# liruiluo/VLA-Adapter

Hardware: AMD Instinct MI355X
Metric: fine-tune samples/sec (224px img + 32-tok prompt), adapter-only, fwd+bwd+AdamW (higher is better)
Workload: dtype bf16

## Files before the change

include/vla_native.h:

```cpp
#ifndef VLA_NATIVE_H
#define VLA_NATIVE_H
#ifdef __cplusplus
extern "C" {
#endif

#define VLA_ERR_ARG (-1)
#define VLA_ERR_LAUNCH (-2)
#define VLA_ERR_UNSUPPORTED (-3)

#define VLA_ABI_VERSION 8
int vla_version(void);
int vla_desc_size(int which);
const char* vla_last_error(void);

enum { VLA_ACT_NONE = 0, VLA_ACT_GELU = 1, VLA_ACT_RELU = 2, VLA_ACT_GELU_TANH = 3, VLA_ACT_SWIGLU = 4, VLA_ACT_SWIGLU_BWD = 5 };

typedef struct vla_gemm_desc {
  const void* A;
  const void* B;
  void* C;
  const void* bias;
  const void* R;
  void* C2;
  int M, N, K, lda, ldb, ldc, ldr, ldc2;
  int res_mod;
  int act, batch;
  long long sA, sB, sC, sR, sC2, sBias;
  float alpha;
  int a_group, c_group;
  long long a_group_stride, c_group_stride;
  int rope_mode, rope_T, rope_dh, rope_cols;
  const float* rope_cos; const float* rope_sin;
  int r_group; long long r_group_stride;
  int c_live_mod, c_live_from;
  int split_k; float* ws;
  int bias_post_round;
  int fp8; const float* a_scale; const float* b_scale;
  const void* A2; const void* B2; int K2, lda2, ldb2;
} vla_gemm_desc;

enum {
  VLA_KERNEL_NT_SKINNY = 0,
  VLA_KERNEL_NT_64x128_S6 = 8,
  VLA_KERNEL_NT_128x128_S4 = 9,
  VLA_KERNEL_NT_128x128 = 10,
  VLA_KERNEL_NT_128x64 = 11,
  VLA_KERNEL_NT_256 = 12,
  VLA_KERNEL_TN_128 = 16,
  VLA_KERNEL_TN_256 = 17
};
int vla_gemm_nt_plan(const vla_gemm_desc* desc , int latency, int num_cus, int* split );
int vla_gemm_latency_hint(int on);
int vla_gemm256_extent_ok(const vla_gemm_desc* desc );
// ... 186 lines not shown
```

vla_adapter_amd/csrc/gemm.hip:

```cpp
#include <algorithm>
#include "gemm_epilogue.h"
#include "gemm_params.h"

namespace {

constexpr int BK = 64;
constexpr int EPI_PAD = 16;

__device__ __forceinline__ float apply_act(float v, int act) {
  switch (act) {
    case VLA_ACT_GELU: return rbf(gelu_erf(v));
    case VLA_ACT_RELU: return fmaxf(v, 0.f);
    case VLA_ACT_GELU_TANH: return rbf(gelu_tanh(v));
    default: return v;
  }
}

template <int BM, int BN, int STAGES, int WN = 2>
struct Cfg {
  static constexpr int NW = (BM / 64) * WN;
  static constexpr int NTHREADS = NW * 64;
  static constexpr int WTN = BN / WN;
  static constexpr int NT = WTN / 16;
  static constexpr int A_BYTES = BM * BK * 2, B_BYTES = BN * BK * 2;
  static constexpr int STAGE_BYTES = A_BYTES + B_BYTES;
  static constexpr int PIECES = STAGE_BYTES / 1024;
  static constexpr int PPW = PIECES / NW;
  static constexpr int EPI_STRIDE = WTN * 2 + EPI_PAD;
  static constexpr int LDS_BYTES = STAGES * STAGE_BYTES;
  static constexpr int NHALF = NW * 64 * EPI_STRIDE <= LDS_BYTES ? 1 : 2;
  static constexpr int EPI_ROWS = 64 / NHALF;
  static constexpr int EPI_BYTES = NW * EPI_ROWS * EPI_STRIDE;
  static_assert(EPI_BYTES <= LDS_BYTES, "epilogue staging must fit the operand ring");
  static_assert(PIECES % NW == 0, "pieces must divide evenly over the waves");
};

template <int BM, int BN, int STAGES, int ROPE, int WN = 2, bool F8 = false, bool EXT = false>
__global__ __launch_bounds__((BM / 64) * 64 * WN) __attribute__((amdgpu_waves_per_eu((F8 && EXT) ? 4 : 1)))
void gemm_nt_kernel(GemmP p) {
  using C = Cfg<BM, BN, STAGES, WN>;
  constexpr int EB = F8 ? 1 : 2;
  extern __shared__ __attribute__((aligned(16))) char smem[];
  const int tid = threadIdx.x, lane = tid & 63;
  const int wid = __builtin_amdgcn_readfirstlane(tid >> 6);
  const int wr = wid / WN, wc = wid - wr * WN;

  const int swz = xcd_order(blockIdx.x, p.ntiles);
  constexpr int GM = 6;
  const int tiles_m = p.ntiles / p.tiles_n, per_group = GM * p.tiles_n;
  const int grp = swz / per_group, rem = swz - grp * per_group;
  const int gm = min(GM, tiles_m - grp * GM);
  const int bm = grp * GM + rem % gm, bn = rem / gm;
  const int m0 = bm * BM, n0 = bn * BN;
  const int z = blockIdx.z;
  const char* Ab = reinterpret_cast<const char*>(p.A) + (long long)z * p.sA * EB;
  const char* Bb = reinterpret_cast<const char*>(p.B) + (long long)z * p.sB * EB;

  const int kc = ((lane & 7) ^ ((lane >> 3) & 7)) * 16;
  const char* pp[C::PPW];
#pragma unroll
  for (int i = 0; i < C::PPW; ++i) {
    const int pc = wid * C::PPW + i;
    if (pc < BM / 8) {
      const int ra = min(m0 + pc * 8 + (lane >> 3), p.M - 1);
      pp[i] = Ab + grouped_row(ra, p.gA, p.sgA, p.lda) * EB + kc;
    } else {
      const int rb = min(n0 + (pc - BM / 8) * 8 + (lane >> 3), p.N - 1);
      pp[i] = Bb + (long long)rb * p.ldb * EB + kc;
    }
  }
  const char* pp2[EXT ? C::PPW : 1];
  if constexpr (EXT) {
#pragma unroll
    for (int i = 0; i < C::PPW; ++i) {
      const int pc = wid * C::PPW + i;
      if (pc < BM / 8) pp2[i] = reinterpret_cast<const char*>(p.A2) + (long long)min(m0 + pc * 8 + (lane >> 3), p.M - 1) * p.lda2 * 2 + kc;
      else pp2[i] = reinterpret_cast<const char*>(p.B2) + (long long)min(n0 + (pc - BM / 8) * 8 + (lane >> 3), p.N - 1) * p.ldb2 * 2 + kc;
    }
  }
  const int nt1 = (p.Ktot > 0 ? min(p.K, p.Ktot - z * p.K) : p.K) / (F8 ? 2 * BK : BK);
  auto stage = [&](int buf, int t) {
    char* base = smem + buf * C::STAGE_BYTES + wid * C::PPW * 1024;
    if (EXT && t >= nt1) {
#pragma unroll
      for (int i = 0; i < C::PPW; ++i) glds16(pp2[i] + (t - nt1) * 128, base + i * 1024);
    } else {
#pragma unroll
      for (int i = 0; i < C::PPW; ++i) glds16(pp[i] + t * 128, base + i * 1024);
    }
  };

  f32x4 acc[C::NT][4];
#pragma unroll
  for (int a = 0; a < C::NT; ++a)
#pragma unroll
    for (int b = 0; b < 4; ++b) acc[a][b] = f32x4{0.f, 0.f, 0.f, 0.f};

  const int frow = lane & 15;
  int foff[2], foff2[2];
#pragma unroll
  for (int s = 0; s < 2; ++s) {
    foff[s] = frow * 128 + (((F8 ? 2 * (lane >> 4) + s : 4 * s + (lane >> 4)) ^ (lane & 7)) << 4);
    foff2[s] = frow * 128 + (((4 * s + (lane >> 4)) ^ (lane & 7)) << 4);
  }

  const int wm0 = m0 + wr * 64, wn0 = n0 + wc * C::WTN;
  const int lq = lane >> 4, lr = lane & 15;
  constexpr bool PERM = ROPE == 1 && C::NT == 2;
  const bool wide = PERM && p.rope_dh == 128;
  auto cbase = [&](int ni) { return PERM ? (wide ? ni * 64 + wc * 16 : (wc >> 1) * 64 + ni * 32 + (wc & 1) * 16) : wc * C::WTN + ni * 16; };
  const bf16_t* bias = p.bias ? p.bias + (long long)z * p.sBias : nullptr;
  float bv[C::NT][4];
  {
    const bool bvec = bias && (((size_t)bias & 7) == 0);
#pragma unroll
    for (int ni = 0; ni < C::NT; ++ni) {
      const int n = n0 + cbase(ni) + lq * 4;
      if (bvec && n + 3 < p.N) {
// ... 37 lines not shown
      _Pragma("unroll") for (int i = 0; i < C::NT; ++i) fn[s][i] = *reinterpret_cast<const bf16x8*>(sb + cbase(i) * 128 + FO[s]);    \
    }                                                                                                                                \
    if constexpr (F8T) {                                                                                                             \
      _Pragma("unroll") for (int ni = 0; ni < C::NT; ++ni)                                                                           \
        _Pragma("unroll") for (int mi = 0; mi < 4; ++mi)                                                                             \
          acc[ni][mi] = __builtin_amdgcn_mfma_scale_f32_16x16x128_f8f6f4(cat8(fn[0][ni], fn[1][ni]), cat8(fm[0][mi], fm[1][mi]),     \
                                                                         acc[ni][mi], 0, 0, 0, 0x7f7f7f7f, 0, 0x7f7f7f7f);            \
    } else {                                                                                                                         \
      _Pragma("unroll") for (int s = 0; s < 2; ++s)                                                                                  \
        _Pragma("unroll") for (int ni = 0; ni < C::NT; ++ni)                                                                         \
          _Pragma("unroll") for (int mi = 0; mi < 4; ++mi)                                                                           \
            acc[ni][mi] = __builtin_amdgcn_mfma_f32_16x16x32_bf16(fn[s][ni], fm[s][mi], acc[ni][mi], 0, 0, 0);                       \
    }                                                                                                                                \
    if (++buf == STAGES) buf = 0;                                                                                                    \
  } while (0)
  if constexpr (F8 && EXT) {
    for (int t = 0; t < nt1; ++t) VLA_KTILE(true, foff);
    {
      float fsa[4];
#pragma unroll
      for (int mi = 0; mi < 4; ++mi) fsa[mi] = p.scaleA[min(wm0 + mi * 16 + lr, p.M - 1)];
#pragma unroll
      for (int ni = 0; ni < C::NT; ++ni)
#pragma unroll
        for (int j = 0; j < 4; ++j) {
          const float sbv = p.scaleB[min(n0 + cbase(ni) + lq * 4 + j, p.N - 1)];
#pragma unroll
          for (int mi = 0; mi < 4; ++mi) acc[ni][mi][j] *= fsa[mi] * sbv;
        }
    }
    for (int t = nt1; t < nt; ++t) VLA_KTILE(false, foff2);
// ... 257 lines not shown
    for (int j = 0; j < 4; ++j) {
      float v = epi_linear(a[j], alpha, bias ? bb[j] : 0.f);
      if (act != VLA_ACT_NONE) v = apply_act(rbf(v), act);
      if (R) v = rbf(v) + rr[j];
      o[j] = v;
    }
    if (vec) {
      *reinterpret_cast<uint2*>(C + (long long)m * ldc + n) = pack4(o);
    } else {
#pragma unroll
      for (int j = 0; j < 4; ++j) C[(long long)m * ldc + n + j] = f2bf(o[j]);
    }
  }
}

template <int BM, int BN, int STAGES, int ROPE, int WN = 2, bool F8 = false, bool EXT = false>
int launch(const GemmP& p0, int nb, hipStream_t st) {
  using C = Cfg<BM, BN, STAGES, WN>;
  if (int rc = vla_lds_limit<gemm_nt_kernel<BM, BN, STAGES, ROPE, WN, F8, EXT>>(C::LDS_BYTES, "gemm_nt_kernel")) return rc;
  GemmP p = p0;
  p.tiles_n = (p.N + BN - 1) / BN;
  p.ntiles = ((p.M + BM - 1) / BM) * p.tiles_n;
  hipLaunchKernelGGL((gemm_nt_kernel<BM, BN, STAGES, ROPE, WN, F8, EXT>), dim3(p.ntiles, 1, nb), dim3(C::NTHREADS), C::LDS_BYTES, st, p);
  return VLA_OK;
}

template <int ROPE, bool F8 = false, bool EXT = false>
int launch_nt(int kernel, const GemmP& p, int nb, hipStream_t st) {
  if constexpr (!F8 && !EXT && ROPE != 3) {
    if (kernel == VLA_KERNEL_NT_64x128_S6) return launch<64, 128, 6, ROPE, 4>(p, nb, st);
    if (kernel == VLA_KERNEL_NT_128x128_S4) return launch<128, 128, 4, ROPE, 4>(p, nb, st);
    if constexpr (ROPE != 1)
      if (kernel == VLA_KERNEL_NT_128x64) return launch<128, 64, 2, ROPE>(p, nb, st);
  }
  return launch<128, 128, 2, ROPE, 4, F8, EXT>(p, nb, st);
}

struct NtOverrides {
// ... 48 lines not shown
      (d->rope_mode == 1 && d->rope_dh != 64) || !vla_gemm256_extent_ok(d))
    return false;
  const unsigned long long ra = (unsigned long long)((d->M + 255) / 256) * 256, rb = (unsigned long long)((d->N + 255) / 256) * 256;
  if ((ra * d->lda2 + d->K2) * 2 >= (1ull << 32) || (rb * d->ldb2 + d->K2) * 2 >= (1ull << 32)) return false;
  if (force != 0) return force == 6;
  const long long t256 = (long long)((d->M + 255) / 256) * ((d->N + 255) / 256);
  if (d->rope_mode == 1 && t256 < 192) return false;
  return use_256(d->M, d->N, d->K + d->K2, 1, d->act, ncu);
}

struct NtPlan { int kernel, split; };

NtPlan plan_nt(const vla_gemm_desc* d, bool latency, int ncu, const NtOverrides& ov) {
  const int force = ov.tile, kt = d->K / BK;
  const int asked = d->split_k > 1 ? d->split_k : 1, per = (kt + asked - 1) / asked, split = (kt + per - 1) / per;
  if (force == 0 && !ov.no_skinny && d->batch == 1 && split == 1 && d->a_group == 0 && d->c_group == 0 && d->r_group == 0 &&
      d->res_mod == 0 && d->c_live_mod == 0 && !d->fp8 && d->K2 == 0 && d->C) {
    const int t = skinny_tile(d, latency, ncu, ov.no_small_rows);
    if (t >= 0) return {VLA_KERNEL_NT_SKINNY + t, 1};
  }
  const bool fits256 = vla_gemm256_extent_ok(d) != 0;
  if (d->K2 > 0) return {!d->fp8 && ext_on_256(d, force, ncu) ? VLA_KERNEL_NT_256 : VLA_KERNEL_NT_128x128, 1};
  if (d->fp8) {
    const bool big = force == 6 || (force == 0 && d->M >= 4096 && d->N >= 4096 && d->K >= 4096);
    return {big && d->c_group == 0 && d->r_group == 0 && fits256 && !(d->rope_mode == 1 && d->rope_dh != 64) ? VLA_KERNEL_NT_256
                                                                                                              : VLA_KERNEL_NT_128x128, 1};
  }
  const int nb = asked > 1 ? asked : d->batch;
  bool square = false;
  if (asked == 1) {
// ... 104 lines not shown
  if (split_k) {
    VLA_REQUIRE(d->ws && d->batch == 1 && d->rope_mode == 0 && d->c_group == 0 && d->r_group == 0 &&
                    d->res_mod == 0 && d->c_live_mod == 0 && d->C &&
                    (d->act == VLA_ACT_NONE || d->act == VLA_ACT_GELU || d->act == VLA_ACT_RELU || d->act == VLA_ACT_GELU_TANH),
                "gemm: split_k needs an fp32 workspace [split_k, M, N], batch 1 and a plain epilogue");
    VLA_REQUIRE(d->N % 4 == 0 && ((uintptr_t)d->ws & 15) == 0, "gemm: split_k needs N % 4 == 0 and a 16-B aligned workspace");
  }
  VLA_REQUIRE(d->c_live_mod >= 0 && d->c_live_from >= 0 && (d->c_live_mod == 0 || d->c_live_from < d->c_live_mod),
              "gemm: c_live_from must lie inside c_live_mod");
  VLA_REQUIRE(d->r_group >= 0 && d->r_group_stride % 8 == 0 && (d->r_group == 0 || d->res_mod == 0),
              "gemm: r_group stride must keep 16-B alignment; r_group and res_mod are exclusive");
  if (d->K2 != 0)
    VLA_REQUIRE(d->K2 > 0 && d->K2 % BK == 0 && d->A2 && d->B2 && d->lda2 % 8 == 0 && d->ldb2 % 8 == 0 && (((uintptr_t)d->A2 | (uintptr_t)d->B2) & 15) == 0 &&
                    d->batch == 1 && !split_k && d->rope_mode != 2,
                "gemm: the K extension needs A2 / B2 (bf16, 16-B aligned rows, K2 % 64 == 0), batch 1, no split-K / interleaved RoPE");
  if (d->rope_mode != 0) {
    VLA_REQUIRE(d->rope_mode == 1 || d->rope_mode == 2, "gemm: rope_mode 0/1/2");
    VLA_REQUIRE(d->rope_cos && d->rope_sin && d->rope_T > 0 && d->rope_dh > 0 && d->rope_dh % 4 == 0 && d->rope_cols % 64 == 0 &&
                    (((uintptr_t)d->rope_cos | (uintptr_t)d->rope_sin) & 15) == 0 && d->act != VLA_ACT_SWIGLU,
                "gemm: bad rope arguments");
    if (d->rope_mode == 1) VLA_REQUIRE(d->rope_dh == 64 || (d->rope_dh == 128 && d->N % 128 == 0 && d->rope_cols % 128 == 0),
                                       "gemm: fused rotate_half RoPE needs head dim 64, or 128 with N and rope_cols multiples of 128");
  }

  const NtOverrides ov = nt_overrides();
  const int ncu = vla_num_cus();
  const NtPlan pl = plan_nt(d, g_latency_hint > 0, ncu, ov);

  GemmP p;
  p.A = (const bf16_t*)d->A; p.B = (const bf16_t*)d->B; p.C = (bf16_t*)d->C;
// ... 2 lines not shown
  p.ldc2 = d->ldc2; p.res_mod = d->res_mod; p.act = d->act;
  p.sA = d->sA; p.sB = d->sB; p.sC = d->sC; p.sR = d->sR; p.sC2 = d->sC2; p.sBias = d->sBias;
  p.tiles_n = p.ntiles = 0; p.batch = 1; p.stagger = 0;
  p.alpha = d->alpha == 0.f ? 1.f : d->alpha;
  p.gA = d->a_group; p.sgA = d->a_group_stride; p.gC = d->c_group; p.sgC = d->c_group_stride;
  p.gR = d->r_group; p.sgR = d->r_group_stride;
  p.c_live_mod = d->c_live_mod; p.c_live_from = d->c_live_from;
  p.bias_post = d->bias_post_round;
  p.ws = nullptr; p.Ktot = 0;
  if (split_k) {
    const int kt = d->K / BK;
    p.ws = d->ws;
    p.K = (kt + pl.split - 1) / pl.split * BK;
    p.Ktot = d->K;
    p.sA = p.sB = p.K;
    p.bias = nullptr; p.R = nullptr;
  }
  p.rope_mode = d->rope_mode; p.rope_T = d->rope_T; p.rope_dh = d->rope_dh; p.rope_cols = d->rope_cols;
  p.rope_cos = d->rope_cos; p.rope_sin = d->rope_sin;
  p.scaleA = d->fp8 ? d->a_scale : nullptr; p.scaleB = d->fp8 ? d->b_scale : nullptr;
  p.A2 = (const bf16_t*)d->A2; p.B2 = (const bf16_t*)d->B2; p.K2 = d->K2; p.lda2 = d->lda2; p.ldb2 = d->ldb2;

  hipStream_t st = (hipStream_t)stream;
  const int nb = pl.split > 1 ? pl.split : d->batch;
  const int rope = d->act == VLA_ACT_SWIGLU_BWD ? 3 : d->rope_mode;
  int rc;
  if (pl.kernel < VLA_KERNEL_NT_SKINNY + SKINNY_TILES) rc = vla_gemm_skinny_launch(p, pl.kernel - VLA_KERNEL_NT_SKINNY, st);
  else if (pl.kernel == VLA_KERNEL_NT_256)
    rc = vla_gemm256_launch(p, d->act == VLA_ACT_SWIGLU ? 1 : d->act == VLA_ACT_SWIGLU_BWD ? 2 : 0, d->batch, ov.grid_set ? ov.grid : ncu, st);
  else if (d->K2 > 0 && d->fp8)
    rc = rope == 3 ? launch_nt<3, true, true>(pl.kernel, p, nb, st) : rope == 1 ? launch_nt<1, true, true>(pl.kernel, p, nb, st)
                                                                                : launch_nt<0, true, true>(pl.kernel, p, nb, st);
  else if (d->K2 > 0)
    rc = rope == 3 ? launch_nt<3, false, true>(pl.kernel, p, nb, st) : rope == 1 ? launch_nt<1, false, true>(pl.kernel, p, nb, st)
                                                                                 : launch_nt<0, false, true>(pl.kernel, p, nb, st);
  else if (d->fp8) rc = rope == 1 ? launch_nt<1, true>(pl.kernel, p, nb, st) : launch_nt<0, true>(pl.kernel, p, nb, st);
  else if (rope == 3) rc = launch_nt<3>(pl.kernel, p, nb, st);
  else if (rope == 2) rc = launch_nt<2>(pl.kernel, p, nb, st);
  else if (rope == 1) rc = launch_nt<1>(pl.kernel, p, nb, st);
  else rc = launch_nt<0>(pl.kernel, p, nb, st);
  if (rc) return rc;
  VLA_CHECK_LAUNCH("gemm_bf16_nt");
  if (pl.split > 1) return splitk_finalize(d, pl.split, st);
  return VLA_OK;
}
```

vla_adapter_amd/engine.py:

```python
from __future__ import annotations

import contextlib
import math
import os
from dataclasses import dataclass, field
from typing import Dict, List, Optional, Tuple

import torch

from . import ops, schedule
from .ops import ACT_GELU, ACT_GELU_TANH, ACT_NONE, ACT_RELU, ACT_SWIGLU, BF16
from .schedule import Segment, capture_graph, chunks, turnaround_chunks

NUM_TOKENS = 64
IGNORE_INDEX = -100


def rup(n: int, m: int) -> int:
    return (n + m - 1) // m * m


def copy_flat(dst: torch.Tensor, src: torch.Tensor):
    n = src.numel()
    ops.copy2d(src, dst, 1, n, n, n)
# ... 557 lines not shown
        assert D % 64 == 0 and (D // self.H) % 8 == 0
        self.D, self.nb, self.Din = D, nb, Da * D
        assert self.Din % 64 == 0
        seg = [("w_adp", (nb, 2 * D, D)), ("b_adp", (nb, 2 * D)),
               ("w_task", (nb, 2 * D, D)), ("b_task", (nb, 2 * D))] if cfg.pro else []
        spec = [("w_x", (nb, 3 * D, D)), ("b_x", (nb, 3 * D))] + seg + [
                ("w_o", (nb, D, D)), ("b_o", (nb, D)), ("w_ffn", (nb, D, D)), ("b_ffn", (nb, D)),
                ("ln_w", (nb, D)), ("ln_b", (nb, D)), ("gate", (nb, 8)),
                ("ln1_w", (self.Din,)), ("ln1_b", (self.Din,)), ("fc1_w", (D, self.Din)), ("fc1_b", (D,)),
                ("ln2_w", (D,)), ("ln2_b", (D,)), ("fc2_w", (Da, D)), ("fc2_b", (Da,)),
                ("p_fc1_w", (D, Pd)), ("p_fc1_b", (D,)), ("p_fc2_w", (D, D)), ("p_fc2_b", (D,)),
                ("action_queries", (NUM_TOKENS, D))]
        self.P = FlatParams(spec, device)
        self.film = {}
        z = lambda *s: torch.zeros(*s, device=device, dtype=BF16)
        self.T = dict(w_x=z(nb, D, 3 * D), w_o=z(nb, D, D), w_ffn=z(nb, D, D), p_fc2_w=z(D, D))
        if cfg.pro:
            self.T.update(w_adp=z(nb, D, 2 * D), w_task=z(nb, D, 2 * D))
        self.fc2T = z(D, 64)
        self.pfc1_pad = z(D, 64)
        self.dirty = True
        self._key = None
        self._prep_key = None
        self.rope_tab = None
        self.ref_softmax = bool(int(os.environ.get("VLA_HEAD_REF_SOFTMAX", "0")))

    _BLK_PRO = [("q_proj", "w_x", "b_x", 0), ("k_self", "w_x", "b_x", 1), ("v_self", "w_x", "b_x", 2),
                ("k_adapter", "w_adp", "b_adp", 0), ("v_adapter", "w_adp", "b_adp", 1),
                ("k_task", "w_task", "b_task", 0), ("v_task", "w_task", "b_task", 1),
                ("o_proj", "w_o", "b_o", 0), ("ffn.1", "w_ffn", "b_ffn", 0)]
    _BLK_ORIG = [("q_proj", "w_x", "b_x", 0), ("k_proj", "w_x", "b_x", 1), ("v_proj", "w_x", "b_x", 2),
                 ("o_proj", "w_o", "b_o", 0), ("ffn.1", "w_ffn", "b_ffn", 0)]

    @property
    def _BLK(self):
        return self._BLK_PRO if self.pro else self._BLK_ORIG

    def _kv(self, which: str, i: int):
        D = self.D
        if self.pro:
            return self.P.view("w_" + which)[i], self.P.view("b_" + which)[i], self.T["w_" + which][i]
        return self.P.view("w_x")[i, D:], self.P.view("b_x")[i, D:], self.T["w_x"][i][:, D:]

    def named_views(self, buf=None) -> Dict[str, torch.Tensor]:
        P, D, out = self.P, self.D, {}
        v = lambda n: P.view(n, buf)
        for i in range(self.nb):
            pre = f"model.mlp_resnet_blocks.{i}."
            for name, w, b, k in self._BLK:
                out[pre + name + ".weight"] = v(w)[i, k * D:(k + 1) * D]
                out[pre + name + ".bias"] = v(b)[i, k * D:(k + 1) * D]
            out[pre + "ffn.0.weight"], out[pre + "ffn.0.bias"] = v("ln_w")[i], v("ln_b")[i]
            out[pre + "gating_factor"] = v("gate")[i, :1]
        for a, b in (("model.layer_norm1.weight", "ln1_w"), ("model.layer_norm1.bias", "ln1_b"), ("model.fc1.weight", "fc1_w"),
                     ("model.fc1.bias", "fc1_b"), ("model.layer_norm2.weight", "ln2_w"), ("model.layer_norm2.bias", "ln2_b"),
                     ("model.fc2.weight", "fc2_w"), ("model.fc2.bias", "fc2_b")):
            out[a] = v(b)
# ... 10 lines not shown
            t.copy_(head_sd[k].to(self.device, BF16).reshape(t.shape))
        for k, t in head_sd.items():
            if "film_gen" in k:
                self.film[k] = t.to(self.device, BF16)
        for k, t in self.proprio_views().items():
            t.copy_(proprio_sd[k].to(self.device, BF16))
        if action_queries is not None:
            self.P.view("action_queries").copy_(action_queries.to(self.device, BF16))
        self.dirty = True

    def head_state_dict(self):
        sd = {k: v.clone() for k, v in self.named_views().items()}
        sd.update(self.film)
        return sd

    @property
    def dirty(self) -> bool:
        return self._stale_fwd or self._stale_bwd

    @dirty.setter
    def dirty(self, v: bool):
        self._stale_fwd = self._stale_bwd = bool(v)

    def refresh_forward_operands(self):
        if self._stale_fwd:
            pd = self.cfg.proprio_dim
            ops.copy2d(self.P.view("p_fc1_w"), self.pfc1_pad, self.D, pd, pd, self.pfc1_pad.stride(0))
            self._stale_fwd = False

    def refresh_transposes(self):
        if not self._stale_bwd:
            return
        P = self.P
        for k in (("w_x", "w_adp", "w_task", "w_o", "w_ffn") if self.pro else ("w_x", "w_o", "w_ffn")):
            ops.transpose(P.view(k), out=self.T[k])
        ops.transpose(P.view("p_fc2_w"), out=self.T["p_fc2_w"])
        ops.transpose(P.view("fc2_w"), out=self.fc2T)
        self._stale_bwd = False

    def _alloc(self, B: int, Kt: int):
        if self._key == (B, Kt):
            return
        before = dict(self.__dict__)
        D, nb, T, dev = self.D, self.nb, self.cfg.chunk, self.device
        Ka = NUM_TOKENS + 1
        e = lambda *s, dt=BF16: torch.empty(*s, device=dev, dtype=dt)
        z = lambda *s, dt=BF16: torch.zeros(*s, device=dev, dtype=dt)
        R = B * T
        self.Ka, self.Kt, self.R = Ka, Kt, R
        self.h_adp = e(nb, B, Ka, D)
        self.KV_adp, self.KV_task = e(nb, B * Ka, 2 * D), e(nb, B * Kt, 2 * D)
        self.dKV_adp, self.dKV_task = e(nb, B * Ka, 2 * D), e(nb, B * Kt, 2 * D)
        self.X = e(nb + 1, R, D)
# ... 55 lines not shown
            assert tuple(noise.shape) == (T, self.Din) and noise.is_contiguous()
            ops.copy2d(noise, self.x_in, B * T, self.Din, self.Din, self.Din, src_mod=T)
        else:
            ops.zero_(self.x_in)
        self.x_ln, self.st1 = ops.layernorm_fwd(self.x_in, P.view("ln1_w"), P.view("ln1_b"), 1e-5, want_stats=True)
        ops.gemm_nt(self.x_ln, P.view("fc1_w"), bias=P.view("fc1_b"), act=ACT_RELU, out=self.X[0])

    def fwd_layer(self, i: int):
        cfg, P, D, H = self.cfg, self.P, self.D, self.H
        HS, B, S, Kt, Ka, T = self.HSref, self.B, self.S, self.Kt, self.Ka, cfg.chunk
        dh = D // H
        rc, rs_ = self.rope_tab
        hs2 = HS[i + 1].view(B * S, D)
        ops.gather_rows(hs2, self.row_idx_ka.view(-1), self.h_adp[i].view(B * Ka, D))
        fuse = self.pro and D % 64 == 0 and not os.environ.get("VLA_NO_KV_ROPE_FUSE")
        wa, ba, _ = self._kv("adp", i)
        ops.gemm_nt(self.h_adp[i].view(B * Ka, D), wa, bias=ba, out=self.KV_adp[i], rope=(2, rc, rs_, Ka, dh, D) if fuse else None)
        wt, bt, _ = self._kv("task", i)
        ops.gemm_nt(hs2[:B * Kt], wt, bias=bt, out=self.KV_task[i], a_group=(Kt, S * D), bias_post_round=B > 1,
                    rope=(2, rc, rs_, Kt, dh, D) if fuse else None)
        x = self.X[i]
        if self.pro:
            if not fuse:
                ops.rope_inter_(self.KV_adp[i][:, :D], rc, rs_, Ka, H, dh, 0)
                ops.rope_inter_(self.KV_task[i][:, :D], rc, rs_, Kt, H, dh, 0)
            ops.gemm_nt(x, P.view("w_x")[i], bias=P.view("b_x")[i], out=self.QKVx[i], rope=(2, rc, rs_, T, dh, 2 * D))
        else:
            ops.gemm_nt(x, P.view("w_x")[i], bias=P.view("b_x")[i], out=self.QKVx[i])
        self._attn(i, fwd=True)
        ops.gemm_nt(self.AOx[i], P.view("w_o")[i], bias=P.view("b_o")[i], residual=x, out=self.O2[i])
        ops.layernorm_fwd(self.O2[i], P.view("ln_w")[i], P.view("ln_b")[i], 1e-5, out=self.LNo[i], stats=self.stats[i])
        ops.gemm_nt(self.LNo[i], P.view("w_ffn")[i], bias=P.view("b_ffn")[i], act=ACT_RELU, out=self.X[i + 1])

# ... 28 lines not shown
            self.bwd_layer(i, dHS)
        self.bwd_end()

    def prep_backward(self, pos1: torch.Tensor, Np: int, B: int, S: int, row0: int, pos0=None, cnt0=None):
        self._alloc(B, Np)
        g = self.guard if pos0 is not None else None
        ops.head_index_prep(pos1, pos0 if pos0 is not None else pos1, cnt0 if cnt0 is not None else pos1, self._idx_scratch,
                            self.row_idx_live_ka, g, B, S, Np, row0)
        self._prep_key = (B, S, Np, row0)

    def bwd_begin(self, dpred: torch.Tensor, row0: int = 0):
        cfg, P, nb = self.cfg, self.P, self.nb
        R, Da = self.R, cfg.action_dim
        self.row0 = row0
        assert self._prep_key == (self.B, self.S, self.Np, row0), "prep_backward() first"
        self.refresh_transposes()
        ops.zero_(self.acc32)
        dp = dpred.reshape(R, Da)
        ops.zero_(self.dpad)
        ops.copy2d(dp, self.dpad, R, Da, Da, 64)
        ops.colsum_(dp, self.b_f32["fc2_b"])
        self._dw(self.dpad, self.xf_ln, out=self.dfc2)
        ops.copy2d(self.dfc2, P.g("fc2_w"), Da, self.D, self.D, self.D)
        d_ln2 = ops.gemm_nt(self.dpad, self.fc2T)
        self.dx = ops.layernorm_bwd(d_ln2, self.X[nb], P.view("ln2_w"), self.st2, self.ln2_dw, self.ln2_db)

    def bwd_layer(self, i: int, dHS: torch.Tensor):
        P, D = self.P, self.D
        B, S, Kt, Ka = self.B, self.S, self.Kt, self.Ka
        dff = self.dFF[i]
        ops.relu_bwd(self.dx, self.X[i + 1], out=dff)
        d_ln = ops.gemm_nt(dff, self.T["w_ffn"][i])
        do2 = self.dO2[i]
        ops.layernorm_bwd(d_ln, self.O2[i], P.view("ln_w")[i], self.stats[i], self.ln_dw[i], self.ln_db[i], out=do2)
        d_ao = ops.gemm_nt(do2, self.T["w_o"][i])
        self._attn(i, fwd=False, dout=d_ao)
        self.dx = ops.gemm_nt(self.dQKVx[i], self.T["w_x"][i], residual=do2)
        ops.gemm_nt(self.dKV_adp[i], self._kv("adp", i)[2], out=self.dh_adp[i])
        ops.scatter_add_rows(self.dh_adp[i], self.row_idx_live_ka.view(-1), dHS[i + 1].view(-1, D))
        if self.row0 == 0:
            ops.gemm_nt(self.dKV_task[i], self._kv("task", i)[2], out=dHS[i + 1].view(B * S, D)[:B * Kt], c_group=(Kt, S * D))

    def bwd_end(self):
        cfg, P, D, nb = self.cfg, self.P, self.D, self.nb
        B, Ka = self.B, self.Ka
        G = P.g
        dy1 = ops.relu_bwd(self.dx, self.X[0])
        ops.colsum_(dy1, self.b_f32["fc1_b"])
        self._dw(dy1, self.x_ln, out=G("fc1_w"))
        d_xln = ops.gemm_nt(dy1, self._t(P.view("fc1_w")))
        ops.layernorm_bwd(d_xln, self.x_in, P.view("ln1_w"), self.st1, self.ln1_dw, self.ln1_db, want_dx=False)
        ops.colsum_(self.dh_adp.view(nb, B, Ka, D)[:, :, NUM_TOKENS].transpose(0, 1), self.d_pf32)
        d_pf = ops.cast_f32_bf16(self.d_pf32)
        ops.colsum_(d_pf, self.b_f32["p_fc2_b"])
        self._dw(d_pf, self.pp_act, out=G("p_fc2_w"))
        d_act = ops.gemm_nt(d_pf, self.T["p_fc2_w"])
        d_pre = ops.gelu_bwd(d_act, self.pp_pre)
        ops.colsum_(d_pre, self.b_f32["p_fc1_b"])
        self._dw(d_pre, self.pr_in, out=self.dpfc1)
        ops.copy2d(self.dpfc1, G("p_fc1_w"), D, cfg.proprio_dim, 64, cfg.proprio_dim)
        Kt, S = self.Kt, self.S
        h_adp = self.h_adp.view(nb, B * Ka, D)
        if self.h_task_c is None:
            h_task, tg = self.HSref[1:nb + 1, 0, :Kt], (Kt, S * D)
        else:
            for i in range(nb):
                ops.copy_rows3d(self.HSref[i + 1], self.h_task_c[i], B, Kt, D, S * D, D, Kt * D, D)
            h_task, tg = self.h_task_c, None
        ops.gemm_tn(self.dQKVx, self.X[:nb], out=G("w_x"))
        ops.gemm_tn(self.dO2, self.AOx, out=G("w_o"))
        ops.gemm_tn(self.dFF, self.LNo, out=G("w_ffn"))
# ... 2 lines not shown
            ops.gemm_tn(self.dKV_adp, h_adp, out=G("w_adp"))
            ops.gemm_tn(self.dKV_task, h_task, out=G("w_task"), rows=B * Kt, b_group=tg)
            ops.colsum_(self.dKV_adp, self.b_f32["b_adp"]); ops.colsum_(self.dKV_task, self.b_f32["b_task"])
        else:
            gkv = G("w_x")[:, self.D:]
            ops.gemm_tn(self.dKV_adp, h_adp, out=gkv, accumulate=True)
            ops.gemm_tn(self.dKV_task, h_task, out=gkv, accumulate=True, rows=B * Kt, b_group=tg)
            bkv = self.b_f32["b_x"][:, self.D:]
            ops.colsum_(self.dKV_adp, bkv); ops.colsum_(self.dKV_task, bkv)
        for k, t in self.b_f32.items():
            ops.cast_f32_bf16(t, out=G(k))
        ops.cast_f32_bf16(self.ln_dw, out=G("ln_w")); ops.cast_f32_bf16(self.ln_db, out=G("ln_b"))
        ops.cast_f32_bf16(self.ln1_dw, out=G("ln1_w")); ops.cast_f32_bf16(self.ln1_db, out=G("ln1_b"))
        ops.cast_f32_bf16(self.ln2_dw, out=G("ln2_w")); ops.cast_f32_bf16(self.ln2_db, out=G("ln2_b"))
        ops.copy2d(self.dgate, G("gate"), nb, 1, 1, 8)

    def _t(self, w2d):
        return ops.transpose(w2d.contiguous())

    def _dw(self, dy, x, out=None):
        return ops.gemm_tn(dy, x, out=out, split=0)


class VLAEngine(schedule.StepControls):

    def __init__(self, cfg: VLACfg, weights: Dict, device="cuda"):
        self.cfg, self.device = cfg, device
        self.vits = [ViT(c, sd, device, j) for j, (c, sd) in enumerate(zip(cfg.vit, weights["vit"]))]
        self.llm = LLM(cfg.llm, weights["llm"], device)
        self.head = Head(cfg, device)
        self.head.load_state_dicts(weights["head"], weights["proprio"], weights.get("action_queries"))
        g = lambda k: weights["proj"][k].to(device=device, dtype=BF16).contiguous()
        self.proj = {k: g(k) for k in weights["proj"]}
# ... 518 lines not shown
            with torch.cuda.stream(hs):
                clip.sumsq(*r_head, gscale)
                head_summed.record(hs)
            clip.sumsq(*r_aq, gscale)
            cur.wait_event(head_summed)
            clip.finalise()
            finalised.record(cur)
            hs.wait_event(finalised)

        def adam(sl):
            args = (self.step_count, lr, beta1, beta2, eps, wd)
            if clip is None:
                ops.adamw_(P.data[sl], P.grad[sl], P.m[sl], P.v[sl], *args, gscale=gscale)
            else:
                ops.adamw_clipped_(P.data[sl], P.grad[sl], P.m[sl], P.v[sl], clip.coef, *args, gscale=gscale)
        with torch.cuda.stream(hs):
            adam(slice(None, aq_off))
            side_done = torch.cuda.Event()
            side_done.record()
        adam(slice(aq_off, None))
        if join:
            cur.wait_event(side_done)
        self.head.dirty = True

    def begin_validation(self):
        self.flush()
        if self._vis_ev is not None:
            torch.cuda.current_stream().wait_event(self._vis_ev)
        self.head.refresh_forward_operands()

    def end_validation(self):
        if self._g_vis is not None:
            self._launch_vision()

    def val_forward(self, batch: Dict[str, torch.Tensor], noise: Optional[torch.Tensor] = None) -> torch.Tensor:
# ... 19 lines not shown
```

vla_adapter_amd/native.py:

```python
from __future__ import annotations

import ctypes as C
import os
from typing import NamedTuple

_HERE = os.path.dirname(os.path.abspath(__file__))
LIB_PATH = (os.environ.get("VLA_NATIVE_LIB") or None) or os.path.join(_HERE, "libvla_native.so")

ACT_NONE, ACT_GELU, ACT_RELU, ACT_GELU_TANH, ACT_SWIGLU, ACT_SWIGLU_BWD = 0, 1, 2, 3, 4, 5
KERNEL_NT_SKINNY, KERNEL_NT_64x128_S6, KERNEL_NT_128x128_S4, KERNEL_NT_128x128, KERNEL_NT_128x64, KERNEL_NT_256 = 0, 8, 9, 10, 11, 12
KERNEL_TN_128, KERNEL_TN_256 = 16, 17
ABI_VERSION = 8


class NativeLibraryMissing(ImportError):
    pass


class GemmDesc(C.Structure):
    _fields_ = [("A", C.c_void_p), ("B", C.c_void_p), ("C", C.c_void_p), ("bias", C.c_void_p), ("R", C.c_void_p),
                ("C2", C.c_void_p),
                ("M", C.c_int), ("N", C.c_int), ("K", C.c_int), ("lda", C.c_int), ("ldb", C.c_int), ("ldc", C.c_int),
                ("ldr", C.c_int), ("ldc2", C.c_int), ("res_mod", C.c_int), ("act", C.c_int), ("batch", C.c_int),
                ("sA", C.c_longlong), ("sB", C.c_longlong), ("sC", C.c_longlong), ("sR", C.c_longlong),
                ("sC2", C.c_longlong), ("sBias", C.c_longlong), ("alpha", C.c_float),
                ("a_group", C.c_int), ("c_group", C.c_int), ("a_group_stride", C.c_longlong), ("c_group_stride", C.c_longlong),
                ("rope_mode", C.c_int), ("rope_T", C.c_int), ("rope_dh", C.c_int), ("rope_cols", C.c_int),
                ("rope_cos", C.c_void_p), ("rope_sin", C.c_void_p),
                ("r_group", C.c_int), ("r_group_stride", C.c_longlong), ("c_live_mod", C.c_int), ("c_live_from", C.c_int),
                ("split_k", C.c_int), ("ws", C.c_void_p), ("bias_post_round", C.c_int),
                ("fp8", C.c_int), ("a_scale", C.c_void_p), ("b_scale", C.c_void_p),
                ("A2", C.c_void_p), ("B2", C.c_void_p), ("K2", C.c_int), ("lda2", C.c_int), ("ldb2", C.c_int)]


class GemmTnDesc(C.Structure):
    _fields_ = [("A", C.c_void_p), ("B", C.c_void_p), ("C", C.c_void_p), ("R", C.c_void_p),
                ("M", C.c_int), ("N1", C.c_int), ("N2", C.c_int), ("lda", C.c_int), ("ldb", C.c_int), ("ldc", C.c_int),
                ("ldr", C.c_int), ("batch", C.c_int),
                ("sA", C.c_longlong), ("sB", C.c_longlong), ("sC", C.c_longlong), ("sR", C.c_longlong), ("alpha", C.c_float),
                ("a_group", C.c_int), ("b_group", C.c_int), ("a_group_stride", C.c_longlong), ("b_group_stride", C.c_longlong),
                ("a_col_group", C.c_int), ("a_col_group_stride", C.c_int), ("split", C.c_int), ("ws", C.c_void_p)]


class AttnDesc(C.Structure):
    _fields_ = [("q", C.c_void_p), ("k", C.c_void_p), ("v", C.c_void_p), ("o", C.c_void_p), ("lse", C.c_void_p),
                ("kmask", C.c_void_p),
                ("q_sb", C.c_longlong), ("k_sb", C.c_longlong), ("v_sb", C.c_longlong), ("o_sb", C.c_longlong),
# ... 211 lines not shown
```

vla_adapter_amd/ops.py:

```python
from __future__ import annotations

import ctypes as C
import math
from typing import Optional, Tuple

import torch

from . import native as N
from .native import ACT_GELU, ACT_GELU_TANH, ACT_NONE, ACT_RELU, ACT_SWIGLU, ACT_SWIGLU_BWD

BF16 = torch.bfloat16


def _lib():
    return N.load()


def _st():
    return C.c_void_p(torch.cuda.current_stream().cuda_stream)


def _p(t: Optional[torch.Tensor]):
    return None if t is None else C.c_void_p(t.data_ptr())


def _chk_bf16(*ts):
    for t in ts:
        if t is not None:
            assert t.is_cuda and t.dtype == BF16, f"expected CUDA bf16 tensor, got {t.device} {t.dtype}"


def gemm_nt(a: torch.Tensor, b: torch.Tensor, *, bias=None, residual=None, res_mod: int = 0, act: int = ACT_NONE,
            out: Optional[torch.Tensor] = None, out2: Optional[torch.Tensor] = None, alpha: float = 1.0,
            want_pre: bool = True, a_group=None, c_group=None, r_group=None, rope=None, c_live=None,
            split_k: Optional[int] = None, bias_post_round: bool = False, fp8=None, ext=None, query_256: bool = False,
            query_plan: bool = False):
    if fp8 is not None:
        assert a.dtype == torch.uint8 and b.dtype == torch.uint8 and a.dim() == 2 and split_k in (None, 0, 1)
        _chk_bf16(bias, residual, out, out2)
        split_k = 0
    else:
        _chk_bf16(a, b, bias, residual, out, out2)
    assert a.stride(-1) == 1 and b.stride(-1) == 1
    batched = a.dim() == 3
    if batched:
        nb, M, K = a.shape
        sA = a.stride(0)
        sB = b.stride(0) if b.dim() == 3 else 0
        Nn = b.shape[-2]
    else:
        nb, (M, K), sA, sB, Nn = 1, a.shape, 0, 0, b.shape[0]
    assert b.shape[-1] == K, f"K mismatch {a.shape} x {b.shape}"
    d = N.GemmDesc()
    d.A, d.B = a.data_ptr(), b.data_ptr()
    d.M, d.N, d.K, d.lda, d.ldb, d.batch = M, Nn, K, a.stride(-2), b.stride(-2), nb
    d.sA, d.sB, d.act, d.alpha, d.res_mod = sA, sB, act, alpha, res_mod
    shape = (nb, M, Nn) if batched else (M, Nn)
    if act == ACT_SWIGLU:
        if out is None and want_pre:
            out = torch.empty(shape, device=a.device, dtype=BF16)
        hshape = shape[:-1] + (Nn // 2,)
        if out2 is None:
            out2 = torch.empty(hshape, device=a.device, dtype=BF16)
        assert out2.shape == hshape and out2.stride(-1) == 1
        d.C2, d.ldc2, d.sC2 = out2.data_ptr(), out2.stride(-2), (out2.stride(0) if batched else 0)
    elif out is None:
        out = torch.empty(shape, device=a.device, dtype=BF16)
    if out is not None:
        assert tuple(out.shape) == tuple(shape) and out.stride(-1) == 1, f"out shape {out.shape} != {shape}"
        d.C, d.ldc, d.sC = out.data_ptr(), out.stride(-2), (out.stride(0) if batched else 0)
    if bias is not None:
# ... 1211 lines not shown
```

Baseline: 1367.

## Read [K,N] weights directly in backward GEMMs via transposing LDS loads

Adds a B_KN variant of the NT GEMM kernel that stages B tiles from a row-major [K, N] weight and uses ds_read_b64_tr_b16 transposing LDS reads to build MFMA operands. Backward data-gradient GEMMs now use the parameter views directly, so the per-step weight transposes and their transposed copies are removed. The b_kn path is pinned to a fixed 128x128 two-stage tile, which bypasses the planner's tile choice and may be slower for some shapes. Separately, the main-stream AdamW slice is now issued before the side-stream slice.

```diff
diff --git a/include/vla_native.h b/include/vla_native.h
--- a/include/vla_native.h
+++ b/include/vla_native.h
@@ -37,6 +37,7 @@
   int bias_post_round;
   int fp8; const float* a_scale; const float* b_scale;
   const void* A2; const void* B2; int K2, lda2, ldb2;
+  int b_kn;
 } vla_gemm_desc;
 
 enum {
diff --git a/vla_adapter_amd/csrc/gemm.hip b/vla_adapter_amd/csrc/gemm.hip
--- a/vla_adapter_amd/csrc/gemm.hip
+++ b/vla_adapter_amd/csrc/gemm.hip
@@ -14,6 +14,19 @@
     case VLA_ACT_GELU_TANH: return rbf(gelu_tanh(v));
     default: return v;
   }
+}
+
+template <int OFF>
+__device__ __forceinline__ bf16x8 lds_read16(unsigned addr) {
+  bf16x8 v;
+  asm volatile("ds_read_b128 %0, %1 offset:%2" : "=v"(v) : "v"(addr), "n"(OFF) : "memory");
+  return v;
+}
+template <int OFF>
+__device__ __forceinline__ bf16x4 lds_read_tr8(unsigned addr) {
+  bf16x4 v;
+  asm volatile("ds_read_b64_tr_b16 %0, %1 offset:%2" : "=v"(v) : "v"(addr), "n"(OFF) : "memory");
+  return v;
 }
 
 template <int BM, int BN, int STAGES, int WN = 2>
@@ -35,10 +48,11 @@
   static_assert(PIECES % NW == 0, "pieces must divide evenly over the waves");
 };
 
-template <int BM, int BN, int STAGES, int ROPE, int WN = 2, bool F8 = false, bool EXT = false>
+template <int BM, int BN, int STAGES, int ROPE, int WN = 2, bool F8 = false, bool EXT = false, bool B_KN = false>
 __global__ __launch_bounds__((BM / 64) * 64 * WN) __attribute__((amdgpu_waves_per_eu((F8 && EXT) ? 4 : 1)))
 void gemm_nt_kernel(GemmP p) {
   using C = Cfg<BM, BN, STAGES, WN>;
+  static_assert(!B_KN || (BN == 128 && ROPE == 0 && !F8 && !EXT), "B as [K, N]: plain bf16 products on 128-column tiles");
   constexpr int EB = F8 ? 1 : 2;
   extern __shared__ __attribute__((aligned(16))) char smem[];
   const int tid = threadIdx.x, lane = tid & 63;
@@ -64,6 +78,9 @@
     if (pc < BM / 8) {
       const int ra = min(m0 + pc * 8 + (lane >> 3), p.M - 1);
       pp[i] = Ab + grouped_row(ra, p.gA, p.sgA, p.lda) * EB + kc;
+    } else if constexpr (B_KN) {
+      const int r = (pc - BM / 8) * 4 + (lane >> 4), f = ((r & 3) << 2) | ((r >> 2) & 3);
+      pp[i] = Bb + ((long long)r * p.ldb + min(n0 + (((lane & 15) ^ f) << 3), p.N - 8)) * 2;
     } else {
       const int rb = min(n0 + (pc - BM / 8) * 8 + (lane >> 3), p.N - 1);
       pp[i] = Bb + (long long)rb * p.ldb * EB + kc;
@@ -84,6 +101,10 @@
     if (EXT && t >= nt1) {
 #pragma unroll
       for (int i = 0; i < C::PPW; ++i) glds16(pp2[i] + (t - nt1) * 128, base + i * 1024);
+    } else if constexpr (B_KN) {
+#pragma unroll
+      for (int i = 0; i < C::PPW; ++i)
+        glds16(pp[i] + (wid * C::PPW + i < BM / 8 ? (long long)t * 128 : (long long)t * BK * p.ldb * 2), base + i * 1024);
     } else {
 #pragma unroll
       for (int i = 0; i < C::PPW; ++i) glds16(pp[i] + t * 128, base + i * 1024);
@@ -102,6 +123,17 @@
   for (int s = 0; s < 2; ++s) {
     foff[s] = frow * 128 + (((F8 ? 2 * (lane >> 4) + s : 4 * s + (lane >> 4)) ^ (lane & 7)) << 4);
     foff2[s] = frow * 128 + (((4 * s + (lane >> 4)) ^ (lane & 7)) << 4);
+  }
+
+  int fbk[B_KN ? C::NT : 1][2];
+  if constexpr (B_KN) {
+    const int kq = lane >> 4, qq = (lane >> 2) & 3, pq = lane & 3;
+#pragma unroll
+    for (int e = 0; e < 2; ++e) {
+      const int row = 8 * kq + qq + 4 * e, f = (qq << 2) | ((2 * kq + e) & 3);
+#pragma unroll
+      for (int i = 0; i < C::NT; ++i) fbk[i][e] = 256 * row + ((((wc * C::WTN + i * 16) >> 3) + (pq >> 1)) ^ f) * 16 + 8 * (pq & 1);
+    }
   }
 
   const int wm0 = m0 + wr * 64, wn0 = n0 + wc * C::WTN;
@@ -169,7 +201,48 @@
     }                                                                                                                                \
     if (++buf == STAGES) buf = 0;                                                                                                    \
   } while (0)
-  if constexpr (F8 && EXT) {
+  if constexpr (B_KN) {
+    static_assert(!B_KN || STAGES == 2, "the [K, N] K loop is written for the two-stage ring");
+    const unsigned lds0 = (unsigned)(size_t)((__attribute__((address_space(3))) char*)smem);
+    for (int t = 0; t < nt; ++t) {
+      asm volatile("s_waitcnt vmcnt(0)" ::: "memory");
+      __builtin_amdgcn_s_barrier();
+      asm volatile("" ::: "memory");
+      if (t + 1 < nt) stage(buf ^ 1, t + 1);
+      const unsigned ua = lds0 + buf * C::STAGE_BYTES + wr * 64 * 128, ub = lds0 + buf * C::STAGE_BYTES + C::A_BYTES;
+      bf16x8 fm[2][4];
+      bf16x4 lo[2][C::NT], hi[2][C::NT];
+#pragma unroll
+      for (int s = 0; s < 2; ++s) {
+        const unsigned a0 = ua + foff[s];
+        fm[s][0] = lds_read16<0>(a0); fm[s][1] = lds_read16<2048>(a0); fm[s][2] = lds_read16<4096>(a0); fm[s][3] = lds_read16<6144>(a0);
+#pragma unroll
+        for (int i = 0; i < C::NT; ++i) {
+          if (s == 0) { lo[s][i] = lds_read_tr8<0>(ub + fbk[i][0]); hi[s][i] = lds_read_tr8<0>(ub + fbk[i][1]); }
+          else { lo[s][i] = lds_read_tr8<8192>(ub + fbk[i][0]); hi[s][i] = lds_read_tr8<8192>(ub + fbk[i][1]); }
+        }
+      }
+#pragma unroll
+      for (int s = 0; s < 2; ++s) {
+        static_assert(C::NT == 2, "the operand lists below name the two n tiles of a 64 x 32 wave tile");
+        if (s == 0)
+          asm volatile("s_waitcnt lgkmcnt(%8)" : "+v"(fm[0][0]), "+v"(fm[0][1]), "+v"(fm[0][2]), "+v"(fm[0][3]), "+v"(lo[0][0]), "+v"(hi[0][0]),
+                       "+v"(lo[0][1]), "+v"(hi[0][1]) : "n"(4 + 2 * C::NT) : "memory");
+        else
+          asm volatile("s_waitcnt lgkmcnt(0)" : "+v"(fm[1][0]), "+v"(fm[1][1]), "+v"(fm[1][2]), "+v"(fm[1][3]), "+v"(lo[1][0]), "+v"(hi[1][0]),
+                       "+v"(lo[1][1]), "+v"(hi[1][1]) : "v"(acc[0][0]), "v"(acc[0][1]), "v"(acc[0][2]), "v"(acc[0][3]), "v"(acc[1][0]),
+                       "v"(acc[1][1]), "v"(acc[1][2]), "v"(acc[1][3]) : "memory");
+        __builtin_amdgcn_sched_barrier(0);
+#pragma unroll
+        for (int ni = 0; ni < C::NT; ++ni) {
+          const bf16x8 fn = {lo[s][ni][0], lo[s][ni][1], lo[s][ni][2], lo[s][ni][3], hi[s][ni][0], hi[s][ni][1], hi[s][ni][2], hi[s][ni][3]};
+#pragma unroll
+          for (int mi = 0; mi < 4; ++mi) acc[ni][mi] = __builtin_amdgcn_mfma_f32_16x16x32_bf16(fn, fm[s][mi], acc[ni][mi], 0, 0, 0);
+        }
+      }
+      buf ^= 1;
+    }
+  } else if constexpr (F8 && EXT) {
     for (int t = 0; t < nt1; ++t) VLA_KTILE(true, foff);
     {
       float fsa[4];
@@ -457,14 +530,14 @@
   }
 }
 
-template <int BM, int BN, int STAGES, int ROPE, int WN = 2, bool F8 = false, bool EXT = false>
+template <int BM, int BN, int STAGES, int ROPE, int WN = 2, bool F8 = false, bool EXT = false, bool B_KN = false>
 int launch(const GemmP& p0, int nb, hipStream_t st) {
   using C = Cfg<BM, BN, STAGES, WN>;
-  if (int rc = vla_lds_limit<gemm_nt_kernel<BM, BN, STAGES, ROPE, WN, F8, EXT>>(C::LDS_BYTES, "gemm_nt_kernel")) return rc;
+  if (int rc = vla_lds_limit<gemm_nt_kernel<BM, BN, STAGES, ROPE, WN, F8, EXT, B_KN>>(C::LDS_BYTES, "gemm_nt_kernel")) return rc;
   GemmP p = p0;
   p.tiles_n = (p.N + BN - 1) / BN;
   p.ntiles = ((p.M + BM - 1) / BM) * p.tiles_n;
-  hipLaunchKernelGGL((gemm_nt_kernel<BM, BN, STAGES, ROPE, WN, F8, EXT>), dim3(p.ntiles, 1, nb), dim3(C::NTHREADS), C::LDS_BYTES, st, p);
+  hipLaunchKernelGGL((gemm_nt_kernel<BM, BN, STAGES, ROPE, WN, F8, EXT, B_KN>), dim3(p.ntiles, 1, nb), dim3(C::NTHREADS), C::LDS_BYTES, st, p);
   return VLA_OK;
 }
 
@@ -543,6 +616,7 @@
 NtPlan plan_nt(const vla_gemm_desc* d, bool latency, int ncu, const NtOverrides& ov) {
   const int force = ov.tile, kt = d->K / BK;
   const int asked = d->split_k > 1 ? d->split_k : 1, per = (kt + asked - 1) / asked, split = (kt + per - 1) / per;
+  if (d->b_kn) return {VLA_KERNEL_NT_128x128, split};
   if (force == 0 && !ov.no_skinny && d->batch == 1 && split == 1 && d->a_group == 0 && d->c_group == 0 && d->r_group == 0 &&
       d->res_mod == 0 && d->c_live_mod == 0 && !d->fp8 && d->K2 == 0 && d->C) {
     const int t = skinny_tile(d, latency, ncu, ov.no_small_rows);
@@ -677,6 +751,8 @@
     VLA_REQUIRE(d->K2 > 0 && d->K2 % BK == 0 && d->A2 && d->B2 && d->lda2 % 8 == 0 && d->ldb2 % 8 == 0 && (((uintptr_t)d->A2 | (uintptr_t)d->B2) & 15) == 0 &&
                     d->batch == 1 && !split_k && d->rope_mode != 2,
                 "gemm: the K extension needs A2 / B2 (bf16, 16-B aligned rows, K2 % 64 == 0), batch 1, no split-K / interleaved RoPE");
+  VLA_REQUIRE(d->b_kn == 0 || (d->b_kn == 1 && !d->fp8 && d->K2 == 0 && d->rope_mode == 0 && d->act != VLA_ACT_SWIGLU_BWD && d->N % 8 == 0),
+              "gemm: b_kn (B as [K, N]) needs N % 8 == 0, bf16 operands and no K extension / RoPE / SwiGLU backward");
   if (d->rope_mode != 0) {
     VLA_REQUIRE(d->rope_mode == 1 || d->rope_mode == 2, "gemm: rope_mode 0/1/2");
     VLA_REQUIRE(d->rope_cos && d->rope_sin && d->rope_T > 0 && d->rope_dh > 0 && d->rope_dh % 4 == 0 && d->rope_cols % 64 == 0 &&
@@ -709,6 +785,7 @@
     p.K = (kt + pl.split - 1) / pl.split * BK;
     p.Ktot = d->K;
     p.sA = p.sB = p.K;
+    if (d->b_kn) p.sB = (long long)p.K * d->ldb;
     p.bias = nullptr; p.R = nullptr;
   }
   p.rope_mode = d->rope_mode; p.rope_T = d->rope_T; p.rope_dh = d->rope_dh; p.rope_cols = d->rope_cols;
@@ -730,6 +807,7 @@
     rc = rope == 3 ? launch_nt<3, false, true>(pl.kernel, p, nb, st) : rope == 1 ? launch_nt<1, false, true>(pl.kernel, p, nb, st)
                                                                                  : launch_nt<0, false, true>(pl.kernel, p, nb, st);
   else if (d->fp8) rc = rope == 1 ? launch_nt<1, true>(pl.kernel, p, nb, st) : launch_nt<0, true>(pl.kernel, p, nb, st);
+  else if (d->b_kn) rc = launch<128, 128, 2, 0, 4, false, false, true>(p, nb, st);
   else if (rope == 3) rc = launch_nt<3>(pl.kernel, p, nb, st);
   else if (rope == 2) rc = launch_nt<2>(pl.kernel, p, nb, st);
   else if (rope == 1) rc = launch_nt<1>(pl.kernel, p, nb, st);
diff --git a/vla_adapter_amd/engine.py b/vla_adapter_amd/engine.py
--- a/vla_adapter_amd/engine.py
+++ b/vla_adapter_amd/engine.py
@@ -595,10 +595,7 @@
         self.P = FlatParams(spec, device)
         self.film = {}
         z = lambda *s: torch.zeros(*s, device=device, dtype=BF16)
-        self.T = dict(w_x=z(nb, D, 3 * D), w_o=z(nb, D, D), w_ffn=z(nb, D, D), p_fc2_w=z(D, D))
-        if cfg.pro:
-            self.T.update(w_adp=z(nb, D, 2 * D), w_task=z(nb, D, 2 * D))
-        self.fc2T = z(D, 64)
+        self.fc2_pad = z(64, D)
         self.pfc1_pad = z(D, 64)
         self.dirty = True
         self._key = None
@@ -620,8 +617,8 @@
     def _kv(self, which: str, i: int):
         D = self.D
         if self.pro:
-            return self.P.view("w_" + which)[i], self.P.view("b_" + which)[i], self.T["w_" + which][i]
-        return self.P.view("w_x")[i, D:], self.P.view("b_x")[i, D:], self.T["w_x"][i][:, D:]
+            return self.P.view("w_" + which)[i], self.P.view("b_" + which)[i]
+        return self.P.view("w_x")[i, D:], self.P.view("b_x")[i, D:]
 
     def named_views(self, buf=None) -> Dict[str, torch.Tensor]:
         P, D, out = self.P, self.D, {}
@@ -662,29 +659,15 @@
         sd.update(self.film)
         return sd
 
-    @property
-    def dirty(self) -> bool:
-        return self._stale_fwd or self._stale_bwd
-
-    @dirty.setter
-    def dirty(self, v: bool):
-        self._stale_fwd = self._stale_bwd = bool(v)
-
     def refresh_forward_operands(self):
-        if self._stale_fwd:
-            pd = self.cfg.proprio_dim
+        if self.dirty:
+            pd, Da = self.cfg.proprio_dim, self.cfg.action_dim
             ops.copy2d(self.P.view("p_fc1_w"), self.pfc1_pad, self.D, pd, pd, self.pfc1_pad.stride(0))
-            self._stale_fwd = False
+            ops.copy2d(self.P.view("fc2_w"), self.fc2_pad, Da, self.D, self.D, self.D)
+            self.dirty = False
 
     def refresh_transposes(self):
-        if not self._stale_bwd:
-            return
-        P = self.P
-        for k in (("w_x", "w_adp", "w_task", "w_o", "w_ffn") if self.pro else ("w_x", "w_o", "w_ffn")):
-            ops.transpose(P.view(k), out=self.T[k])
-        ops.transpose(P.view("p_fc2_w"), out=self.T["p_fc2_w"])
-        ops.transpose(P.view("fc2_w"), out=self.fc2T)
-        self._stale_bwd = False
+        self.refresh_forward_operands()
 
     def _alloc(self, B: int, Kt: int):
         if self._key == (B, Kt):
@@ -770,9 +753,9 @@
         hs2 = HS[i + 1].view(B * S, D)
         ops.gather_rows(hs2, self.row_idx_ka.view(-1), self.h_adp[i].view(B * Ka, D))
         fuse = self.pro and D % 64 == 0 and not os.environ.get("VLA_NO_KV_ROPE_FUSE")
-        wa, ba, _ = self._kv("adp", i)
+        wa, ba = self._kv("adp", i)
         ops.gemm_nt(self.h_adp[i].view(B * Ka, D), wa, bias=ba, out=self.KV_adp[i], rope=(2, rc, rs_, Ka, dh, D) if fuse else None)
-        wt, bt, _ = self._kv("task", i)
+        wt, bt = self._kv("task", i)
         ops.gemm_nt(hs2[:B * Kt], wt, bias=bt, out=self.KV_task[i], a_group=(Kt, S * D), bias_post_round=B > 1,
                     rope=(2, rc, rs_, Kt, dh, D) if fuse else None)
         x = self.X[i]
@@ -831,7 +814,6 @@
         R, Da = self.R, cfg.action_dim
         self.row0 = row0
         assert self._prep_key == (self.B, self.S, self.Np, row0), "prep_backward() first"
-        self.refresh_transposes()
         ops.zero_(self.acc32)
         dp = dpred.reshape(R, Da)
         ops.zero_(self.dpad)
@@ -839,7 +821,7 @@
         ops.colsum_(dp, self.b_f32["fc2_b"])
         self._dw(self.dpad, self.xf_ln, out=self.dfc2)
         ops.copy2d(self.dfc2, P.g("fc2_w"), Da, self.D, self.D, self.D)
-        d_ln2 = ops.gemm_nt(self.dpad, self.fc2T)
+        d_ln2 = ops.gemm_nt(self.dpad, self.fc2_pad, b_kn=True)
         self.dx = ops.layernorm_bwd(d_ln2, self.X[nb], P.view("ln2_w"), self.st2, self.ln2_dw, self.ln2_db)
 
     def bwd_layer(self, i: int, dHS: torch.Tensor):
@@ -847,16 +829,16 @@
         B, S, Kt, Ka = self.B, self.S, self.Kt, self.Ka
         dff = self.dFF[i]
         ops.relu_bwd(self.dx, self.X[i + 1], out=dff)
-        d_ln = ops.gemm_nt(dff, self.T["w_ffn"][i])
+        d_ln = ops.gemm_nt(dff, P.view("w_ffn")[i], b_kn=True)
         do2 = self.dO2[i]
         ops.layernorm_bwd(d_ln, self.O2[i], P.view("ln_w")[i], self.stats[i], self.ln_dw[i], self.ln_db[i], out=do2)
-        d_ao = ops.gemm_nt(do2, self.T["w_o"][i])
+        d_ao = ops.gemm_nt(do2, P.view("w_o")[i], b_kn=True)
         self._attn(i, fwd=False, dout=d_ao)
-        self.dx = ops.gemm_nt(self.dQKVx[i], self.T["w_x"][i], residual=do2)
-        ops.gemm_nt(self.dKV_adp[i], self._kv("adp", i)[2], out=self.dh_adp[i])
+        self.dx = ops.gemm_nt(self.dQKVx[i], P.view("w_x")[i], residual=do2, b_kn=True)
+        ops.gemm_nt(self.dKV_adp[i], self._kv("adp", i)[0], out=self.dh_adp[i], b_kn=True)
         ops.scatter_add_rows(self.dh_adp[i], self.row_idx_live_ka.view(-1), dHS[i + 1].view(-1, D))
         if self.row0 == 0:
-            ops.gemm_nt(self.dKV_task[i], self._kv("task", i)[2], out=dHS[i + 1].view(B * S, D)[:B * Kt], c_group=(Kt, S * D))
+            ops.gemm_nt(self.dKV_task[i], self._kv("task", i)[0], out=dHS[i + 1].view(B * S, D)[:B * Kt], c_group=(Kt, S * D), b_kn=True)
 
     def bwd_end(self):
         cfg, P, D, nb = self.cfg, self.P, self.D, self.nb
@@ -865,13 +847,13 @@
         dy1 = ops.relu_bwd(self.dx, self.X[0])
         ops.colsum_(dy1, self.b_f32["fc1_b"])
         self._dw(dy1, self.x_ln, out=G("fc1_w"))
-        d_xln = ops.gemm_nt(dy1, self._t(P.view("fc1_w")))
+        d_xln = ops.gemm_nt(dy1, P.view("fc1_w"), b_kn=True)
         ops.layernorm_bwd(d_xln, self.x_in, P.view("ln1_w"), self.st1, self.ln1_dw, self.ln1_db, want_dx=False)
         ops.colsum_(self.dh_adp.view(nb, B, Ka, D)[:, :, NUM_TOKENS].transpose(0, 1), self.d_pf32)
         d_pf = ops.cast_f32_bf16(self.d_pf32)
         ops.colsum_(d_pf, self.b_f32["p_fc2_b"])
         self._dw(d_pf, self.pp_act, out=G("p_fc2_w"))
-        d_act = ops.gemm_nt(d_pf, self.T["p_fc2_w"])
+        d_act = ops.gemm_nt(d_pf, P.view("p_fc2_w"), b_kn=True)
         d_pre = ops.gelu_bwd(d_act, self.pp_pre)
         ops.colsum_(d_pre, self.b_f32["p_fc1_b"])
         self._dw(d_pre, self.pr_in, out=self.dpfc1)
@@ -904,9 +886,6 @@
         ops.cast_f32_bf16(self.ln1_dw, out=G("ln1_w")); ops.cast_f32_bf16(self.ln1_db, out=G("ln1_b"))
         ops.cast_f32_bf16(self.ln2_dw, out=G("ln2_w")); ops.cast_f32_bf16(self.ln2_db, out=G("ln2_b"))
         ops.copy2d(self.dgate, G("gate"), nb, 1, 1, 8)
-
-    def _t(self, w2d):
-        return ops.transpose(w2d.contiguous())
 
     def _dw(self, dy, x, out=None):
         return ops.gemm_tn(dy, x, out=out, split=0)
@@ -1455,11 +1434,11 @@
                 ops.adamw_(P.data[sl], P.grad[sl], P.m[sl], P.v[sl], *args, gscale=gscale)
             else:
                 ops.adamw_clipped_(P.data[sl], P.grad[sl], P.m[sl], P.v[sl], clip.coef, *args, gscale=gscale)
+        adam(slice(aq_off, None))
         with torch.cuda.stream(hs):
             adam(slice(None, aq_off))
             side_done = torch.cuda.Event()
             side_done.record()
-        adam(slice(aq_off, None))
         if join:
             cur.wait_event(side_done)
         self.head.dirty = True
diff --git a/vla_adapter_amd/native.py b/vla_adapter_amd/native.py
--- a/vla_adapter_amd/native.py
+++ b/vla_adapter_amd/native.py
@@ -30,7 +30,8 @@
                 ("r_group", C.c_int), ("r_group_stride", C.c_longlong), ("c_live_mod", C.c_int), ("c_live_from", C.c_int),
                 ("split_k", C.c_int), ("ws", C.c_void_p), ("bias_post_round", C.c_int),
                 ("fp8", C.c_int), ("a_scale", C.c_void_p), ("b_scale", C.c_void_p),
-                ("A2", C.c_void_p), ("B2", C.c_void_p), ("K2", C.c_int), ("lda2", C.c_int), ("ldb2", C.c_int)]
+                ("A2", C.c_void_p), ("B2", C.c_void_p), ("K2", C.c_int), ("lda2", C.c_int), ("ldb2", C.c_int),
+                ("b_kn", C.c_int)]
 
 
 class GemmTnDesc(C.Structure):
diff --git a/vla_adapter_amd/ops.py b/vla_adapter_amd/ops.py
--- a/vla_adapter_amd/ops.py
+++ b/vla_adapter_amd/ops.py
@@ -34,7 +34,7 @@
             out: Optional[torch.Tensor] = None, out2: Optional[torch.Tensor] = None, alpha: float = 1.0,
             want_pre: bool = True, a_group=None, c_group=None, r_group=None, rope=None, c_live=None,
             split_k: Optional[int] = None, bias_post_round: bool = False, fp8=None, ext=None, query_256: bool = False,
-            query_plan: bool = False):
+            query_plan: bool = False, b_kn: bool = False):
     if fp8 is not None:
         assert a.dtype == torch.uint8 and b.dtype == torch.uint8 and a.dim() == 2 and split_k in (None, 0, 1)
         _chk_bf16(bias, residual, out, out2)
@@ -47,14 +47,14 @@
         nb, M, K = a.shape
         sA = a.stride(0)
         sB = b.stride(0) if b.dim() == 3 else 0
-        Nn = b.shape[-2]
+        Nn = b.shape[-1 if b_kn else -2]
     else:
-        nb, (M, K), sA, sB, Nn = 1, a.shape, 0, 0, b.shape[0]
-    assert b.shape[-1] == K, f"K mismatch {a.shape} x {b.shape}"
+        nb, (M, K), sA, sB, Nn = 1, a.shape, 0, 0, b.shape[1 if b_kn else 0]
+    assert b.shape[-2 if b_kn else -1] == K, f"K mismatch {a.shape} x {b.shape}"
     d = N.GemmDesc()
     d.A, d.B = a.data_ptr(), b.data_ptr()
     d.M, d.N, d.K, d.lda, d.ldb, d.batch = M, Nn, K, a.stride(-2), b.stride(-2), nb
-    d.sA, d.sB, d.act, d.alpha, d.res_mod = sA, sB, act, alpha, res_mod
+    d.sA, d.sB, d.act, d.alpha, d.res_mod, d.b_kn = sA, sB, act, alpha, res_mod, int(b_kn)
     shape = (nb, M, Nn) if batched else (M, Nn)
     if act == ACT_SWIGLU:
         if out is None and want_pre:
```

Result: no change. 1370 (median of 6 runs) (+0.2%).
